# author-hidden-name/GAN-segmentation

Hardware: AMD Instinct MI355X
Metric: synthetic (image,mask) pairs/sec, FFHQ-1024 StyleGAN+decoder (higher is better)
Workload: dtype f32; 1 GPU; stylegan-ffhq 1024^2 synthesis + 2-class decoder, batch=8 per GPU, fp32 (BASELINE.json configs[1]); synthetic weights/latents/noise; (img u8, mask u8) resident on rank 0; global_batch=8, parallelism=dp1, gather=none, backend=none, graph=eager (GSA_GRAPH=0)

## Files before the change

### gan-segmentation_amd/csrc/gsa_api.cpp

```cpp
#include <hip/hip_runtime.h>

#include <cmath>
#include <cstdarg>
#include <cstdio>
#include <cstdlib>
#include <cstring>
#include <map>
#include <string>
#include <vector>

#include "../../include/gsa.h"
#include "gsa_kernels.h"
#include "gsa_pack.h"

using namespace gsa;

namespace {

constexpr int kMaxLevels = 12;
thread_local std::string g_create_error;

struct HostTensor {
    std::vector<float> data;
    std::vector<int64_t> dims;
// ... 64 lines not shown
    int d_n = 0, d_s0 = 0, d_bn = 1;
    int d_feat[kMaxLevels + 1] = {0}, d_inch[kMaxLevels] = {0};
    std::map<std::string, HostTensor> dparams;
    DecLevelDev dl[kMaxLevels];

    int max_batch = 0;
    float* lat[2] = {nullptr, nullptr};
    float* styles = nullptr;
    float *t_raw = nullptr, *x1 = nullptr;
    float* x2[kMaxLevels] = {nullptr};
    Aff* aff1 = nullptr;
    Aff* aff2[kMaxLevels] = {nullptr};
    StatPart* partials = nullptr;
    StatPart* stat_acc = nullptr;
    unsigned* stat_tickets = nullptr;
    unsigned* map_ctl = nullptr;
    unsigned long long* map_ll[2] = {nullptr, nullptr};
    float* zeros = nullptr;
    unsigned long long* stamps = nullptr;
    float* din[kMaxLevels] = {nullptr};
    float* cvt[kMaxLevels] = {nullptr};
    float *ya[kMaxLevels] = {nullptr}, *scb[kMaxLevels] = {nullptr}, *prev[kMaxLevels] = {nullptr};

    hipStream_t side = nullptr;
    hipEvent_t ev_level[kMaxLevels] = {nullptr};
    hipEvent_t ev_fork = nullptr, ev_join = nullptr;
    int bf16 = 0;
    int prio = 0;
    int dbg = 0;
    int side_levels = -1;
// ... 261 lines not shown
int gsa_create(int device, gsa_ctx** out) {
    if (!out) return fail(nullptr, GSA_ERR_INVALID, "gsa_create: out is null");
    int count = 0;
    hipError_t e = hipGetDeviceCount(&count);
    if (e != hipSuccess || count <= 0)
        return fail(nullptr, GSA_ERR_HIP, "no HIP device available (%s)", e == hipSuccess ? "device count is 0" : hipGetErrorString(e));
    if (device < 0 || device >= count) return fail(nullptr, GSA_ERR_INVALID, "device %d out of range (%d devices)", device, count);
    e = hipSetDevice(device);
    if (e != hipSuccess) return fail(nullptr, GSA_ERR_HIP, "hipSetDevice(%d): %s", device, hipGetErrorString(e));
    gsa_ctx* c = new gsa_ctx();
    c->device = device;
    e = hipStreamCreateWithFlags(&c->side, hipStreamNonBlocking);
    for (int i = 0; e == hipSuccess && i < kMaxLevels; ++i) e = hipEventCreateWithFlags(&c->ev_level[i], hipEventDisableTiming);
    if (e == hipSuccess) e = hipEventCreateWithFlags(&c->ev_fork, hipEventDisableTiming);
    if (e == hipSuccess) e = hipEventCreateWithFlags(&c->ev_join, hipEventDisableTiming);
    if (e != hipSuccess) {
        const int rc = fail(nullptr, GSA_ERR_HIP, "creating the side stream: %s", hipGetErrorString(e));
        delete c;
        return rc;
    }
    if (e == hipSuccess) e = hipMalloc((void**)&c->zeros, 256);
    if (e == hipSuccess) e = hipMemset(c->zeros, 0, 256);
    if (e != hipSuccess) {
        const int rc = fail(nullptr, GSA_ERR_HIP, "allocating the zero page: %s", hipGetErrorString(e));
        delete c;
        return rc;
    }
    c->side_levels = env_int("GSA_SIDE_LEVELS", c->side_levels);
    c->dbg = env_int("GSA_DBG", c->dbg);
    c->prio = env_int("GSA_PRIO", c->prio);
// ... 1 lines not shown
    return GSA_OK;
}

void gsa_destroy(gsa_ctx* c) {
    if (!c) return;
    (void)hipSetDevice(c->device);
    (void)hipDeviceSynchronize();
    free_all(c->g_allocs);
    free_all(c->d_allocs);
    free_all(c->ws_allocs);
    for (auto& ev : c->prof_events) { (void)hipEventDestroy(ev.a); (void)hipEventDestroy(ev.b); }
    for (auto e : c->event_pool) (void)hipEventDestroy(e);
    for (int i = 0; i < kMaxLevels; ++i) if (c->ev_level[i]) (void)hipEventDestroy(c->ev_level[i]);
    if (c->ev_fork) (void)hipEventDestroy(c->ev_fork);
    if (c->ev_join) (void)hipEventDestroy(c->ev_join);
    if (c->side) (void)hipStreamDestroy(c->side);
    if (c->zeros) (void)hipFree(c->zeros);
    delete c;
}

const char* gsa_last_error(const gsa_ctx* c) { return c ? c->err.c_str() : g_create_error.c_str(); }


int gsa_generator_init(gsa_ctx* c, const gsa_generator_config* g) {
    if (!c || !g) return GSA_ERR_INVALID;
    if (g->max_res_log2 < 2 || g->max_res_log2 > kMaxLevels) return fail(c, GSA_ERR_INVALID, "max_res_log2 %d out of range", g->max_res_log2);
    if (g->latent_size != 512) return fail(c, GSA_ERR_INVALID, "latent_size must be 512 (latent_avg is (512,) in the reference)");
    if (g->channels < 1 || g->channels > 4) return fail(c, GSA_ERR_INVALID, "channels must be 1..4");
    c->gc = *g;
    c->nlev = g->max_res_log2 - 1;
// ... 303 lines not shown
            for (int nb = 1; nb <= max_batch; ++nb)
                prow_elems = std::max(prow_elems, (size_t)conv_stat_rows((int)R, (int)R, (int)C, nb) * C);
            prow_elems = std::max(prow_elems, (size_t)post_prow((int)R, (int)R, (int)C) * C);
        }
        if (int rc = dev_alloc(c, N * maxact, &c->t_raw, T)) return rc;
        if (int rc = dev_alloc(c, N * maxact, &c->x1, T)) return rc;
        if (int rc = dev_alloc(c, N * maxC, &c->aff1, T)) return rc;
        prow_elems = std::max(prow_elems, (size_t)64 * maxC);
        if (int rc = dev_alloc_zeroed(c, N * prow_elems, &c->partials, T)) return rc;
        c->partials_bytes = N * prow_elems * sizeof(StatPart);
        c->stat_acc_bytes = N * maxC * sizeof(StatPart);
        c->ticket_bytes = N * ((maxC + 63) / 64) * sizeof(unsigned);
        c->stats_dirty = false;
        if (int rc = dev_alloc_zeroed(c, N * maxC, &c->stat_acc, T)) return rc;
        if (int rc = dev_alloc_zeroed(c, N * ((maxC + 63) / 64), &c->stat_tickets, T)) return rc;
    }
    if (int rc = dev_alloc_zeroed(c, 16, &c->stamps, T)) return rc;
    if (c->d_ready) {
        for (int i = c->d_s0; i < c->d_n; ++i) {
            const DecLevelDev& d = c->dl[i];
            const size_t R = (size_t)4 << i;
            if (int rc = dev_alloc(c, N * R * R * d.I, &c->din[i], T)) return rc;
            if (int rc = dev_alloc(c, N * R * R * d.F, &c->cvt[i], T)) return rc;
            if (!d.is_last) {
                if (int rc = dev_alloc(c, N * 4 * R * R * d.cs, &c->ya[i], T)) return rc;
                if (int rc = dev_alloc(c, N * 4 * R * R * d.cs, &c->prev[i], T)) return rc;
                if (d.has_sc)
                    if (int rc = dev_alloc(c, N * (2 * R >= 16 ? 1 : 4) * R * R * d.cs, &c->scb[i], T)) return rc;
            }
        }
// ... 35 lines not shown
        if (int rc = run_mapping(c, s, n, z, c->lat[0])) return rc;
        const float* w = c->lat[0];
        Launch lp(c, s, "g.styles", 2.0 * N * L * c->style_cols, 4.0 * ((double)L * c->style_cols + N * c->style_cols));
        HIP_TRY(launch_styles(w, c->latent_avg, c->psi, c->style_wt, c->style_b, c->style_col_layer, c->styles, n, L, c->style_cols, s));
    } else {
        Launch lp(c, s, "g.styles", 2.0 * N * L * c->style_cols, 4.0 * ((double)L * c->style_cols + N * 2 * nlev * L + N * c->style_cols));
        HIP_TRY(launch_styles_dlatents(dl, c->latent_avg, c->psi, c->style_wt, c->style_b, c->style_tiles, c->style_num_tiles, c->styles, n, L,
                                       c->style_cols, 2 * nlev, s));
    }

    char layer[64];
    for (int l = 0; l < nlev; ++l) {
        const GenBlockDev& B = c->blk[l];
        const int R = B.R, C = B.C, Cin = B.Cin;
        const double px = N * R * R;
        for (int k = 0; k < 2; ++k) {
            const float* nz = noise[2 * l + k];
            if (!nz) return fail(c, GSA_ERR_INVALID, "noise plane %d is null", 2 * l + k);
            int prow = 0;
            if (k == 0) {
                PostParams pp{};
                pp.noise = nz; pp.nscale = B.nscale[0]; pp.nbias = B.nbias[0];
                pp.out = c->x1; pp.partials = c->partials; pp.H = R; pp.W = R; pp.C = C; pp.bf16 = c->bf16;
                if (!B.has_conv1) {
                    pp.src = c->constant; pp.src_per_sample = 0; pp.blur = nullptr;
                } else {
                    ConvParams cp = conv_base(c);
                    cp.src0 = c->x2[l - 1]; cp.aff0 = c->aff2[l - 1]; cp.C0 = Cin;
                    cp.Hs = R / 2; cp.Ws = R / 2; cp.H = R; cp.W = R;
                    cp.wpk = B.w1; cp.Cout = C; cp.out = c->t_raw;
// ... 9 lines not shown
                    }
                    pp.src = c->t_raw; pp.src_per_sample = 1; pp.blur = B.blur;
                }
                snprintf(layer, sizeof layer, "g.%d.post_1", R);
                if (post_fuses_finalize(pp)) {
                    FinalizeParams fp{};
                    fp.partials = c->partials; fp.prow = 0; fp.HW = R * R; fp.C = C; fp.acc = c->stat_acc; fp.tickets = c->stat_tickets;
                    fp.style = c->styles + B.style_off[0]; fp.style_stride = c->style_cols;
                    fp.gamma = B.gamma[0]; fp.beta = B.beta[0];
                    fp.aff = c->aff1;
                    fp.flags = c->map_ctl;
                    Launch lp(c, s, layer, 0.0, 4.0 * (2 * px * C + px));
                    HIP_TRY(launch_post_fin(pp, fp, n, s));
                    continue;
                }
                Launch lp(c, s, layer, 0.0, 4.0 * (2 * px * C + px));
#ifdef GSA_DBG_HOOKS
                if (!((c->dbg & 8) && R >= 512))
#endif
                HIP_TRY(launch_post(pp, n, s));
                prow = post_rows_used(pp);
            } else {
                ConvParams cp = conv_base(c);
                cp.src0 = c->x1; cp.aff0 = c->aff1; cp.C0 = C;
                cp.Hs = R; cp.Ws = R; cp.H = R; cp.W = R;
                cp.wpk = B.w2; cp.wino = B.w2u; cp.Cout = C; cp.out = c->x2[l];
                cp.noise = nz; cp.nscale = B.nscale[1]; cp.nbias = B.nbias[1]; cp.partials = c->partials;
                snprintf(layer, sizeof layer, "g.%d.conv_2", R);
                int rows = conv_stat_rows(R, R, C, n);
                cp.stat_rows_host = &rows;
                const bool fused_fin = conv_fuses_finalize(cp, EPI_SYNTH, false);
                const double products = conv_form_products(conv3x3_form(cp, EPI_SYNTH, false));
                if (fused_fin) {
                    cp.fin_style = c->styles + B.style_off[1]; cp.fin_style_stride = c->style_cols;
                    cp.fin_gamma = B.gamma[1]; cp.fin_beta = B.beta[1]; cp.fin_aff = c->aff2[l]; cp.fin_flags = c->map_ctl;
                }
                Launch lp(c, s, layer, 2.0 * px * C * C * products, 4.0 * (2 * px * C + px), 2.0 * px * C * C * 9);
                HIP_TRY(launch_conv3x3(cp, EPI_SYNTH, false, n, s));
                prow = rows;
                if (fused_fin) continue;
            }
            if (c->fault == 2 && l == 3 && k == 1) {
// ... 214 lines not shown
    const float* fsrc[kMaxLevels];
    const Aff* faff[kMaxLevels];
    for (int l = 0; l < c->nlev; ++l) { fsrc[l] = c->x2[l]; faff[l] = c->aff2[l]; }
    const int want = c->side_levels < 0 ? c->d_n - 1 : c->side_levels;
    const int ns = want > c->d_n - 1 ? c->d_n - 1 : want;
    if (ns > 0) {
        HIP_TRY(hipEventRecord(c->ev_fork, s));
        HIP_TRY(hipStreamWaitEvent(c->side, c->ev_fork, 0));
    }
    bool fuse_rgb = false;
    if (img && ns <= c->d_n - 1 && factor == 1) {
        const int last = c->d_n - 1;
        ConvParams cp = cvt_params(c, last, fsrc[last], faff[last]);
        fuse_rgb = conv_fuses_torgb(cp, EPI_DEC, false, c->gc.channels);
    }
    if (int rc = run_generator(c, s, n, z, dl, noise, nullptr, fuse_rgb || factor > 1 ? nullptr : img, nullptr, ns > 0)) return rc;
    if (img && factor > 1) {
        const int l = c->nlev - 1, R = c->blk[l].R, C = c->blk[l].C, nc = c->gc.channels;
        const double px = (double)n * R * R;
        Launch lp(c, s, "g.torgb_down", 2.0 * px * C * nc, px * 4.0 * C + px / (factor * factor) * nc);
        HIP_TRY(launch_torgb_down(c->x2[l], c->aff2[l], c->rgb_w, c->rgb_b, img, n, R, R, C, nc, factor, c->bf16, s));
    }
    if (ns > 0) {
        if (int rc = run_decoder(c, c->side, n, fsrc, faff, nullptr, nullptr, 0, ns, true)) return rc;
        HIP_TRY(hipEventRecord(c->ev_join, c->side));
        HIP_TRY(hipStreamWaitEvent(s, c->ev_join, 0));
    }
    return run_decoder(c, s, n, fsrc, faff, nullptr, mask, ns, -1, false, fuse_rgb ? img : nullptr, factor);
}

int gsa_generate(gsa_ctx* c, void* stream, int32_t n, const float* z, const float* const* noise, int32_t num_noise, uint8_t* img,
// ... 135 lines not shown
```

### gan-segmentation_amd/csrc/gsa_dev.h

```cpp
#pragma once
#include "gsa_kernels.h"

#ifndef GSA_NO_XCD_REMAP
#define GSA_NO_XCD_REMAP 0
#endif

namespace gsa {

#ifdef GSA_STAMP
#define GSA_DBG_HOOKS 1
#endif
#ifdef GSA_STAMP
#define STAMP(i) do { __builtin_amdgcn_sched_barrier(0); asm volatile("s_memtime %0\n\ts_waitcnt lgkmcnt(0)" : "=s"(stamp_t[i]) :: "memory"); __builtin_amdgcn_sched_barrier(0); } while (0)
#define STAMP_DECL unsigned long long stamp_t[8] = {0, 0, 0, 0, 0, 0, 0, 0}
#define STAMP_FLUSH(nph) do { if (p.stamps && (threadIdx.x & 63) == 0) { for (int i_ = 0; i_ < (nph); ++i_) atomicAdd(&p.stamps[i_], stamp_t[i_ + 1] - stamp_t[i_]); atomicAdd(&p.stamps[15], 1ull); } } while (0)
#define TICK(var) do { __builtin_amdgcn_sched_barrier(0); asm volatile("s_memtime %0\n\ts_waitcnt lgkmcnt(0)" : "=s"(var) :: "memory"); __builtin_amdgcn_sched_barrier(0); } while (0)
#define TSUM(acc, a, b) acc += (b) - (a)
#define TFLUSH(idx, acc) do { if (p.stamps && (threadIdx.x & 63) == 0) atomicAdd(&p.stamps[idx], acc); } while (0)
#else
#define TICK(var) do {} while (0)
#define TSUM(acc, a, b) do {} while (0)
#define TFLUSH(idx, acc) do {} while (0)
#define STAMP(i) do {} while (0)
#define STAMP_DECL do {} while (0)
#define STAMP_FLUSH(nph) do {} while (0)
#endif


constexpr int kDirectRows = 64;

typedef float f32x4 __attribute__((ext_vector_type(4)));
typedef float f32x2 __attribute__((ext_vector_type(2)));
typedef __bf16 bf16x2 __attribute__((ext_vector_type(2)));
typedef unsigned u32x4 __attribute__((ext_vector_type(4)));
typedef short s16x4 __attribute__((ext_vector_type(4)));


__device__ __forceinline__ float max1(float a, float b) { float r; asm("v_max_f32 %0, %1, %2" : "=v"(r) : "v"(a), "v"(b)); return r; }
__device__ __forceinline__ float lrelu(float v) { return max1(v, 0.2f * v); }

__device__ __forceinline__ unsigned long long to_fixed(float v, double scale) {
    const double magic = 6755399441055744.0;
    double t = fma((double)v, scale, magic);
    return (unsigned long long)__double_as_longlong(t) - (unsigned long long)__double_as_longlong(magic);
}

__device__ __forceinline__ int stat_s2(int HW) {
    const int s2 = 40 - (HW > 1 ? 32 - __builtin_clz((unsigned)HW - 1u) : 0);
    return s2 < 20 ? 20 : (s2 > 26 ? 26 : s2);
}
__device__ __forceinline__ double stat_scale2(int HW) { return __hiloint2double((1023 + stat_s2(HW)) << 20, 0); }
__device__ __forceinline__ unsigned long long to_fixed_sq(float q, int s2) {
    const bool big = q >= __int_as_float((127 + 50 - s2) << 23);
    const float qs = big ? q * __int_as_float((127 + 20 - s2) << 23) : q;
    const unsigned long long k = to_fixed(qs, __hiloint2double((1023 + s2) << 20, 0));
    return k << (big ? s2 - 20 : 0);
}

template <int CTRL>
__device__ __forceinline__ float dpp_quad(float v) {
    return __int_as_float(__builtin_amdgcn_mov_dpp(__float_as_int(v), CTRL, 0xF, 0xF, true));
}

__device__ __forceinline__ f32x4 quad_transpose(float v0, float v1, float v2, float v3, int j) {
    const bool b0 = (j & 1) != 0, b1 = (j & 2) != 0;
    float pa = dpp_quad<0xB1>(v0), pb = dpp_quad<0xB1>(v1);
    const float a0 = b0 ? pb : v0, a1 = b0 ? v1 : pa;
    pa = dpp_quad<0xB1>(v2); pb = dpp_quad<0xB1>(v3);
    const float a2 = b0 ? pb : v2, a3 = b0 ? v3 : pa;
    pa = dpp_quad<0x4E>(a0); pb = dpp_quad<0x4E>(a2);
    const float c0 = b1 ? pb : a0, c2 = b1 ? a2 : pa;
// ... 113 lines not shown
```

### gan-segmentation_amd/csrc/gsa_kernels.h

```cpp
#pragma once
#include <hip/hip_runtime.h>
#include <stdint.h>
#include <stdlib.h>

#include <atomic>
#include <string>

namespace gsa {

struct Aff { float mean, A, B, pad; };

struct StatPart { unsigned long long s1, s2; };

constexpr double kStatScale1 = 268435456.0;

enum Epilogue { EPI_RAW = 0, EPI_SYNTH = 1, EPI_DEC = 2 };

struct ConvParams {
    int device;
    const float* src0; const Aff* aff0; int C0;
    const float* src1; int C1;
    int Hs, Ws;
    int up;
    int H, W;
    const float* wpk;
    const float* wino;
    int Cout;
// ... 4 lines not shown
    const float* resid; int resid_up;
    const float* resid1; int res_c0;
    const float* wsc; const float* sc_bias; float* out_sc;
    int tiles_x, tiles_y, groups, total_tiles;
    int stats_direct;
    int* stat_rows_host;
    int w_resident;
    int group_minor;
    unsigned long long* stamps;
    int dbg;
    int prio;
    int bf16;
    const float* fin_style; int fin_style_stride; const float* fin_gamma; const float* fin_beta; Aff* fin_aff; unsigned* fin_flags;
    const float* zeros;
    const float* rgb_w; const float* rgb_b; uint8_t* rgb_img;
};

struct PostParams {
    const float* src;
    int src_per_sample;
    const float* blur;
    const float* noise; const float* nscale; const float* nbias;
    float* out; StatPart* partials; int prow;
    int H, W, C;
    int bf16;
    int row_groups;
};

struct FinalizeParams {
    const StatPart* partials; int prow; int HW; int C;
// ... 12 lines not shown


enum class ConvForm { Wino43, WinoDma, WinoTwoTiles, WinoLean, Wino, KSplit, Bf16Lean, Direct };
ConvForm conv3x3_form(const ConvParams& p, int epi, bool shortcut);
hipError_t launch_conv3x3(const ConvParams& p, int epi, bool shortcut, int n, hipStream_t s);
inline bool conv_form_wino(ConvForm f) { return f <= ConvForm::Wino; }
inline double conv_form_products(ConvForm f) { return f == ConvForm::Wino43 ? 2.25 : conv_form_wino(f) ? 4 : 9; }
inline bool wino_shape(int H, int Cout, int bf16) { return !bf16 && (H >= 64 || (H >= 32 && Cout >= 64) || (H >= 16 && Cout >= 256)); }
inline bool wino43_shape(int H, int Cin) { return Cin >= 64 && H >= 32; }
bool wino43_enabled();
bool wino_lean_applies(const ConvParams& p, int epi);
bool wino_stream_paired(const ConvParams& p, int n);
hipError_t launch_wino_lean(const ConvParams& p, int epi, int n, hipStream_t s);
bool wino_lean_fuses_torgb(const ConvParams& p, int epi, int nc);
bool conv_fuses_torgb(const ConvParams& p, int epi, bool shortcut, int nc);
bool bf16_lean_applies(const ConvParams& p, int epi, bool shortcut);
hipError_t launch_bf16_lean(const ConvParams& p, int epi, int n, hipStream_t s);
bool subpixel_lean_applies(const ConvParams& p, int nt, int epi, bool sc, int kb, bool wst);
hipError_t launch_subpixel_lean(const ConvParams& q, int nt, int epi, bool sc, int kb, bool wst, dim3 grid, hipStream_t s);
enum class SubPath { Resident, Streamed, Plain };
struct SubpixelPlan {
    int ct;
    SubPath path;
    bool wino;
    int kb;
    size_t lds;
    int wgs_per_group;
};
SubpixelPlan subpixel_plan(const ConvParams& p, bool shortcut, int n);
hipError_t launch_subpixel(const ConvParams& p, int epi, bool shortcut, int n, hipStream_t s);
// ... 82 lines not shown
```

### gan-segmentation_amd/csrc/gsa_kernels.hip

```cpp
#include "gsa_kernels.h"
#include "gsa_dev.h"

#include <cxxabi.h>

#include <cstdio>
#include <cstdlib>
#include <cstring>
#include <mutex>
#include <vector>

#ifndef GSA_MFMA_PRIO
#define GSA_MFMA_PRIO 2
#endif
#ifndef GSA_OPERAND_PIPELINE
#define GSA_OPERAND_PIPELINE 1
#endif
#ifndef GSA_NO_XCD_REMAP
#define GSA_NO_XCD_REMAP 0
#endif
#ifndef GSA_POST_OCC
#define GSA_POST_OCC 2
#endif
#ifndef GSA_WINO_SOA
#define GSA_WINO_SOA 0
// ... 2648 lines not shown
    if ((int)gridDim.x > p.prow) {
        for (int i = threadIdx.x; i < p.C; i += 256) {
            StatPart* a = p.partials + ((size_t)n * p.prow + (blockIdx.x & (kDirectRows - 1))) * p.C + i;
            atomicAdd(&a->s1, sstat[i]);
            atomicAdd(&a->s2, sstat[p.C + i]);
        }
        return;
    }
    for (int i = threadIdx.x; i < p.C; i += 256) {
        StatPart sp; sp.s1 = sstat[i]; sp.s2 = sstat[p.C + i];
        p.partials[((size_t)n * p.prow + blockIdx.x) * p.C + i] = sp;
    }
}

__device__ __forceinline__ void finalize_one(const FinalizeParams& p, int n, int c, unsigned long long I1, unsigned long long I2) {
    const double inv_hw = 1.0 / (double)p.HW;
    const double m = (double)(long long)I1 * (1.0 / kStatScale1) * inv_hw;
    const double e2 = (double)(long long)I2 * (1.0 / stat_scale2(p.HW)) * inv_hw;
    double var = fma(-m, m, e2);
    {
        const long long s1 = (long long)I1;
        const bool near_wrap = (s1 < 0 ? -s1 : s1) >= (1ll << 61) || I2 >= (1ull << 61);
        if (p.flags && (near_wrap || var < -1e-6 * (e2 + m * m) - 1e-30)) atomicOr(p.flags, 1u);
    }
    if (!(var > 0.0)) var = 0.0;
    const float mean_f = (float)m, var_f = (float)var;
    const float inv = 1.0f / sqrtf(var_f + 1e-5f);
    const float gsc = p.gamma[c] * inv;
    const float* st = p.style + (size_t)n * p.style_stride;
    const float s1 = st[c] + 1.0f;
    Aff a;
    a.mean = mean_f;
    a.A = gsc * s1;
    a.B = fmaf(-mean_f, a.A, fmaf(p.beta[c], s1, st[p.C + c]));
    a.pad = 0.0f;
    p.aff[(size_t)n * p.C + c] = a;
}

__global__ __launch_bounds__(256) void finalize_kernel(FinalizeParams p, int rows_per_block) {
    __shared__ unsigned long long sh[2][256];
    __shared__ int is_last;
    const int n = blockIdx.y;
    const int cblk = p.C >= 64 ? 64 : p.C, nrg = 256 / cblk;
    const int cl = threadIdx.x % cblk, rg = threadIdx.x / cblk;
    const int c = blockIdx.x * 64 + cl;
    unsigned long long I1 = 0, I2 = 0;
    if (rg < nrg && c < p.C) {
        const int r0 = blockIdx.z * rows_per_block;
        const int r1 = min(p.prow, r0 + rows_per_block);
        const StatPart* base = p.partials + (size_t)n * p.prow * p.C + c;
#pragma unroll 16
// ... 928 lines not shown
}

ConvForm conv3x3_form(const ConvParams& p, int epi, bool sc) {
    if (wino_rule(p, epi, sc)) {
        if (wino43_enabled() && wino43_shape(p.H, p.C0) && p.resid == nullptr) return ConvForm::Wino43;
        if (wino_dma(p, epi) && wino_nt(p) == 1) return ConvForm::WinoDma;
        if (wino_tw(p) == 2) return ConvForm::WinoTwoTiles;
        return wino_lean_applies(p, epi) ? ConvForm::WinoLean : ConvForm::Wino;
    }
    if (ksplit_rule(p, sc)) return ConvForm::KSplit;
    return bf16_lean_applies(p, epi, sc) ? ConvForm::Bf16Lean : ConvForm::Direct;
}

hipError_t launch_conv3x3(const ConvParams& p, int epi, bool sc, int n, hipStream_t s) {
    if (p.H != p.W || (p.H & (p.H - 1)) || p.H < 4 || p.Cout % 16 || p.C0 % 16 || p.C1 % 16) return hipErrorInvalidValue;
    switch (conv3x3_form(p, epi, sc)) {
#if GSA_EXPERIMENTS
        case ConvForm::Wino43: return launch_wino43(p, epi, n, s);
        case ConvForm::WinoDma: return launch_wino_dma(p, epi, n, s);
        case ConvForm::WinoTwoTiles: return launch_wino_two_tiles(p, epi, n, s);
#endif
        case ConvForm::WinoLean: return launch_wino_lean(p, epi, n, s);
        case ConvForm::Wino: return launch_wino(p, epi, n, s);
        case ConvForm::KSplit: return launch_ksplit(p, epi, n, s);
        case ConvForm::Bf16Lean: return launch_bf16_lean(p, epi, n, s);
        case ConvForm::Direct: return launch_direct(p, epi, sc, n, s);
        default: return hipErrorInvalidValue;
    }
}

static bool fuse_finalize() {
    static const bool enabled = env_int("GSA_FUSEFIN", 1) != 0;
    return enabled;
}
bool conv_fuses_finalize(const ConvParams& p, int epi, bool sc) {
    return fuse_finalize() && epi == EPI_SYNTH && p.H <= 8 && conv3x3_form(p, epi, sc) == ConvForm::KSplit;
}

bool conv_fuses_torgb(const ConvParams& p, int epi, bool sc, int nc) {
    return conv3x3_form(p, epi, sc) == ConvForm::WinoLean && wino_lean_fuses_torgb(p, epi, nc);
}

bool subpixel_uses_wino(const ConvParams& p) {
    static const bool enabled = env_int("GSA_WINO22", 1) != 0;
    return enabled && !p.bf16;
}

SubpixelPlan subpixel_plan(const ConvParams& p, bool sc, int n) {
    static const bool res_enabled = env_int("GSA_SUBRES", 1) != 0;
    static const bool wst_enabled = env_int("GSA_SUBWST", 1) != 0;
    SubpixelPlan plan{};
    plan.wino = subpixel_uses_wino(p);
    const long tiles = (long)(p.H / 16) * (p.W / 16) * n;
    plan.ct = 16;
    for (int ct = plan.wino ? 32 : 64; ct > 16; ct /= 2)
// ... 270 lines not shown
```

### gan-segmentation_amd/csrc/gsa_wino_lean.hip

```cpp
#include "gsa_kernels.h"
#include "gsa_dev.h"

#include <cstdio>
#include <cstdlib>
#include <type_traits>

namespace gsa {
namespace lean {

constexpr int LH = 18, LW = 18, RS = LW * 16 + 4;
constexpr int IMG = LH * RS;
constexpr int SEG = 16 * 256;
constexpr int NPIX = LH * LW;

struct Tile { int n, y0, x0; };

template <int EPI, bool AFF, bool RES, int NB, int GW, bool DB = true, int PF = 1, bool RGB = false>
__global__ __launch_bounds__(256 * GW, GW == 1 ? (DB ? 2 : 3) : 1) void conv3x3_wino_lean(ConvParams p) {
    static_assert(!RGB || (NB == 1 && GW == 1 && DB && AFF && EPI == EPI_DEC), "fused toRGB: the 16 -> 16 decoder kernel with an AdaIN source");
    static_assert(DB || (NB == 1 && GW == 1), "single-buffered form: one block, one group");
    static_assert(PF == 1 || (PF == 2 && DB), "two prefetch sets: the double-buffered form");
    constexpr int NTHR = 256 * GW, CIN = 16 * NB, COUT = 16 * GW;
    constexpr int NCH = (NPIX * 4 + NTHR - 1) / NTHR;
    constexpr bool kLastPartial = (NPIX * 4) % NTHR != 0;
    extern __shared__ __attribute__((aligned(16))) float smem[];
    float* const sA = smem;
    float* const sB = smem + (DB ? 2 : 1) * IMG;
    const int tid = threadIdx.x, lane = tid & 63;
    const int wave8 = __builtin_amdgcn_readfirstlane(tid >> 6);
    const int wave = wave8 & 3, gsel = wave8 >> 2;
    const int i16 = lane & 15, kq = lane >> 4, part = tid & 3;
    const int H = p.H, W = p.W;
    const int per = (p.total_tiles + (int)gridDim.x - 1) / (int)gridDim.x;
    const int w_begin = xcd_block(blockIdx.x, gridDim.x) * per;
    const int w_end = min(p.total_tiles, w_begin + per);
    if (w_begin >= w_end) return;
// ... 37 lines not shown
        if (e) {
#pragma unroll
            for (int k = 0; k < NCH; ++k) {
                const unsigned bad = (eflags >> (4 * k)) & (unsigned)e;
                const unsigned off = s_off[k] + (bad ? safe_off - s_off[k] : 0u);
                ra[S][k] = *reinterpret_cast<const f32x4*>(hb + off);
            }
        } else {
#pragma unroll
            for (int k = 0; k < NCH; ++k) ra[S][k] = *reinterpret_cast<const f32x4*>(hb + s_off[k]);
        }
    };
    auto write_item = [&](auto set_tag, const Tile& t, int e, int cb, int buf) {
        constexpr int S = decltype(set_tag)::value;
        float* img = sA + buf * IMG;
        if (AFF && t.n != n_coef) {
#pragma unroll
            for (int h = 0; h < NB; ++h) {
                const f32x4* a = reinterpret_cast<const f32x4*>(p.aff0 + (size_t)t.n * CIN + h * 16 + part * 4);
                const f32x4 a0 = a[0], a1 = a[1], a2 = a[2], a3 = a[3];
                cA[h] = f32x4{a0[1], a1[1], a2[1], a3[1]};
                cB[h] = f32x4{a0[2], a1[2], a2[2], a3[2]};
            }
            n_coef = t.n;
        }
        const f32x4 kA = NB == 1 || cb == 0 ? cA[0] : cA[NB - 1], kB = NB == 1 || cb == 0 ? cB[0] : cB[NB - 1];
        const f32x4 z = {0.f, 0.f, 0.f, 0.f};
        if (e) {
#pragma unroll
            for (int k = 0; k < NCH; ++k) {
                const f32x4 v = AFF ? fma4(ra[S][k], kA, kB) : ra[S][k];
// ... 268 lines not shown
            __syncthreads();
            if (has_next) write_item(S0{}, tr, er, 0, 0);
            epilogue_loads(tc);
            Tile t2 = tr; int e2c = er, cb2 = 0;
            if (it + 2 < items) { next_item(t2, e2c, cb2); load_item(S0{}, t2, e2c, cb2); }
            mfmas(std::true_type{}, 0);
            loads_landed(ra[0], acc[15]);
            epilogue(tc);
            if (EPI == EPI_SYNTH && (!has_next || tr.n != tc.n)) flush_stats(tc.n);
            __syncthreads();
            tc = tr; ec = er; tr = t2; er = e2c;
        }
    }
}

__device__ unsigned g_cu_tickets[4096];
__device__ __forceinline__ void antiphase_start(int cycles64, float* lds_word) {
    if (cycles64 <= 0) return;
    if (threadIdx.x == 0) {
        unsigned hw, xcc;
        asm volatile("s_getreg_b32 %0, hwreg(HW_REG_HW_ID)" : "=s"(hw));
        asm volatile("s_getreg_b32 %0, hwreg(HW_REG_XCC_ID)" : "=s"(xcc));
        const unsigned cu = ((xcc & 15u) << 8) | (((hw >> 13) & 7u) << 5) | (((hw >> 12) & 1u) << 4) | ((hw >> 8) & 15u);
        *reinterpret_cast<unsigned*>(lds_word) = atomicAdd(&g_cu_tickets[cu & 4095u], 1u);
    }
    __syncthreads();
    const unsigned ticket = *reinterpret_cast<volatile unsigned*>(lds_word);
    __syncthreads();
    if (ticket & 1u)
        for (int i = 0; i < cycles64; i += 16) __builtin_amdgcn_s_sleep(16);
}

template <int EPI, bool AFF, int NT, int IL, bool PAIR>
__device__ __forceinline__ void wino_stream_body(const ConvParams& p) {
    static_assert(!PAIR || (NT == 1 && IL == 0), "paired form: one group per wave quad, phased memory instructions");
    constexpr int NTHR = PAIR ? 512 : 256;
    constexpr int NCH = (NPIX * 4 + NTHR - 1) / NTHR;
    constexpr int NP = PAIR ? 2 : NT;
    extern __shared__ __attribute__((aligned(16))) float smem[];
    float* const sA = smem;
    float* const sB = smem + 2 * IMG;
    float* const sE = sB + 2 * NP * SEG;
    float* const sC = sE + 64 * NP;
    const int tid = threadIdx.x, lane = tid & 63;
    const int wave8 = __builtin_amdgcn_readfirstlane(tid >> 6);
    const int wave = PAIR ? wave8 & 3 : wave8;
    const int quad = PAIR ? wave8 >> 2 : 0;
    const int i16 = lane & 15, kq = lane >> 4, part = tid & 3;
    const int H = p.H, W = p.W, CIN = p.C0, COUT = p.Cout, nblk = p.C0 >> 4;
    const int g = PAIR ? 2 * (int)blockIdx.y + quad : (int)blockIdx.y;
// ... 47 lines not shown
        if ((p.dbg & 512) && dbg_items > 2) return;
#endif
        if (e) {
#pragma unroll
            for (int k = 0; k < NCH; ++k) {
                const unsigned bad = (eflags >> (4 * k)) & (unsigned)e;
                const unsigned off = s_off[k] + (bad ? safe_off - s_off[k] : 0u);
                ra[k] = *reinterpret_cast<const f32x4*>(hb + off);
            }
        } else {
#pragma unroll
            for (int k = 0; k < NCH; ++k) ra[k] = *reinterpret_cast<const f32x4*>(hb + s_off[k]);
        }
    };
    int n_coef = -1;
    auto coefficients = [&](int n) {
        __syncthreads();
        for (int e = tid; e < CIN; e += NTHR) {
            const f32x4 a = *reinterpret_cast<const f32x4*>(p.aff0 + (size_t)n * CIN + e);
            sC[(e >> 4) * 32 + (e & 15)] = a[1];
            sC[(e >> 4) * 32 + 16 + (e & 15)] = a[2];
        }
        __syncthreads();
    };
    auto write_item = [&](const Tile& t, int e, int cb, int buf) {
        float* img = sA + buf * IMG;
        if (AFF && t.n != n_coef) { coefficients(t.n); n_coef = t.n; }
#ifdef GSA_DBG_HOOKS
        if (++dbg_items > 2 && (p.dbg & 128)) return;
#endif
        f32x4 kA = {0.f, 0.f, 0.f, 0.f}, kB = kA;
        if (AFF) {
            kA = *reinterpret_cast<const f32x4*>(sC + cb * 32 + part * 4);
            kB = *reinterpret_cast<const f32x4*>(sC + cb * 32 + 16 + part * 4);
        }
        const f32x4 z = {0.f, 0.f, 0.f, 0.f};
        if (e) {
#pragma unroll
            for (int k = 0; k < NCH; ++k) {
                const f32x4 v = AFF ? fma4(ra[k], kA, kB) : ra[k];
                const bool bad = ((eflags >> (4 * k)) & (unsigned)e) != 0;
                if (k < NCH - 1 || l_off[NCH - 1] >= 0) *reinterpret_cast<f32x4*>(img + l_off[k]) = bad ? z : v;
// ... 243 lines not shown
    }
    TFLUSH(6, sw); TFLUSH(7, sl); TFLUSH(8, sm); TFLUSH(9, se); TFLUSH(10, sb);
    TFLUSH(12, (unsigned long long)items); TFLUSH(15, 1ull);
}

template <int EPI, bool AFF, int NT = 1, int IL = 0>
__global__ __launch_bounds__(256, NT == 1 ? 2 : 1) void conv3x3_wino_stream(ConvParams p) {
    wino_stream_body<EPI, AFF, NT, IL, false>(p);
}

template <int EPI, bool AFF>
__global__ __launch_bounds__(512, 1) void conv3x3_wino_stream_pair(ConvParams p) {
    wino_stream_body<EPI, AFF, 1, 0, true>(p);
}

template <int EPI, bool AFF, bool RES, int NB, int GW, bool DB = true, int PF = 1, bool RGB = false>
hipError_t launch_t(const ConvParams& p, int n, hipStream_t s) {
    const size_t lds = sizeof(float) * ((DB ? 2 : 1) * IMG + GW * NB * SEG);
    const int cus = device_cus(p.device);
    ConvParams q = p;
    q.wpk = p.wino;
    q.tiles_x = p.W / 16;
    q.tiles_y = p.H / 16;
    q.groups = 1;
    q.total_tiles = q.tiles_x * q.tiles_y * n;
    if (EPI == EPI_SYNTH) {
        q.stats_direct = 1;
        q.prow = kDirectRows;
        if (p.stat_rows_host) *p.stat_rows_host = q.prow;
    }
    const int gx = std::min(q.total_tiles, cus * (GW == 1 ? (DB ? 2 : 3) : 1));
    return launch<conv3x3_wino_lean<EPI, AFF, RES, NB, GW, DB, PF, RGB>>(p.device, dim3(gx), dim3(256 * GW), lds, s, q);
}

bool single_buffered() {
    static const bool on = env_int("GSA_WINO_LEAN_SB", 0) != 0;
    return on;
}

int prefetch_sets() {
    static const int pf = env_int("GSA_WINO_LEAN_PF", 1);
    return pf == 2 ? 2 : 1;
}

template <int NB, int GW>
hipError_t launch_shape(const ConvParams& p, int epi, int n, hipStream_t s) {
// ... 37 lines not shown
    q.groups = p.Cout / (16 * NP);
#if GSA_EXPERIMENTS
    static const int stagger = env_int("GSA_STAGGER", 0);
    q.group_minor = PAIR ? 0 : stagger;
#else
    q.group_minor = 0;
#endif
    q.total_tiles = q.tiles_x * q.tiles_y * n;
    if (EPI == EPI_SYNTH) {
        q.stats_direct = 1;
        q.prow = kDirectRows;
        if (p.stat_rows_host) *p.stat_rows_host = q.prow;
    }
    const int slots = std::max(1, cus * (NP == 1 ? 2 : 1) / q.groups);
    const int gx = std::min(q.total_tiles, slots);
    if constexpr (PAIR) return launch<conv3x3_wino_stream_pair<EPI, AFF>>(p.device, dim3(gx, q.groups), dim3(512), lds, s, q);
    else return launch<conv3x3_wino_stream<EPI, AFF, NT, IL>>(p.device, dim3(gx, q.groups), dim3(256), lds, s, q);
}

}
using namespace lean;

bool wino_lean_applies(const ConvParams& p, int epi) {
    static const int enabled = env_int("GSA_WINO_LEAN", 7);
    if (p.H != p.W || p.H % 16) return false;
    if ((enabled & 4) && p.C0 >= 64 && p.C0 <= 512 && p.resid == nullptr && p.H >= 16)
        return epi == EPI_SYNTH ? (p.partials != nullptr && p.noise != nullptr && p.fin_aff == nullptr) : epi == EPI_DEC;
    const bool shape = (p.C0 == 16 && p.Cout == 16 && (enabled & 1)) || (p.C0 == 32 && p.Cout == 32 && (enabled & 2));
    if (!shape || p.H < 32) return false;
    if (epi == EPI_SYNTH) return p.partials != nullptr && p.noise != nullptr && p.fin_aff == nullptr && p.resid == nullptr;
// ... 24 lines not shown
#else
    (void)p; (void)n;
    return false;
#endif
}

int stream_interleaved() {
#if GSA_EXPERIMENTS
    static const int il = env_int("GSA_WINO_IL", 0);
    return il == 1 ? 1 : 0;
#else
    return 0;
#endif
}

hipError_t launch_wino_lean(const ConvParams& p, int epi, int n, hipStream_t s) {
    if (p.C0 >= 64) {
#if GSA_EXPERIMENTS
        if (stream_pairs(p, n)) {
            const int il = stream_interleaved();
#define GSA_STREAM2(IL_) \
            if (il == IL_) { \
                if (epi == EPI_SYNTH) return p.aff0 ? launch_stream_t<EPI_SYNTH, true, 2, IL_>(p, n, s) : launch_stream_t<EPI_SYNTH, false, 2, IL_>(p, n, s); \
                if (epi == EPI_DEC) return p.aff0 ? launch_stream_t<EPI_DEC, true, 2, IL_>(p, n, s) : launch_stream_t<EPI_DEC, false, 2, IL_>(p, n, s); \
                return hipErrorInvalidValue; \
            }
            GSA_STREAM2(0) GSA_STREAM2(1)
#undef GSA_STREAM2
            return hipErrorInvalidValue;
        }
#endif
// ... 16 lines not shown
```

Measured before the change: 1424 pairs/s.

## Fuse AdaIN stat finalization into the following Winograd conv for synth conv_2

For generator levels of 64 and up, the post kernel after conv_1 now writes per-sample statistic rows to a dedicated zeroed buffer. The next Winograd conv reduces those rows in LDS and computes the AdaIN affine coefficients itself, so the separate finalize step between the two convolutions is skipped. The buffer is zeroed on a side stream at call start and the main stream waits on an event before first use. The cost is redundant reduction work in every workgroup whenever the tile's sample changes, plus extra LDS atomics and kernel variants.

```diff
diff --git a/gan-segmentation_amd/csrc/gsa_api.cpp b/gan-segmentation_amd/csrc/gsa_api.cpp
--- a/gan-segmentation_amd/csrc/gsa_api.cpp
+++ b/gan-segmentation_amd/csrc/gsa_api.cpp
@@ -102,6 +102,12 @@
     StatPart* partials = nullptr;
     StatPart* stat_acc = nullptr;
     unsigned* stat_tickets = nullptr;
+    StatPart* rows1[kMaxLevels] = {nullptr};
+    StatPart* sum_rows = nullptr;
+    size_t sum_rows_bytes = 0;
+    hipEvent_t ev_rows = nullptr;
+    bool sums_call = false;
+    bool sums_wait = false;
     unsigned* map_ctl = nullptr;
     unsigned long long* map_ll[2] = {nullptr, nullptr};
     float* zeros = nullptr;
@@ -393,6 +399,7 @@
     for (int i = 0; e == hipSuccess && i < kMaxLevels; ++i) e = hipEventCreateWithFlags(&c->ev_level[i], hipEventDisableTiming);
     if (e == hipSuccess) e = hipEventCreateWithFlags(&c->ev_fork, hipEventDisableTiming);
     if (e == hipSuccess) e = hipEventCreateWithFlags(&c->ev_join, hipEventDisableTiming);
+    if (e == hipSuccess) e = hipEventCreateWithFlags(&c->ev_rows, hipEventDisableTiming);
     if (e != hipSuccess) {
         const int rc = fail(nullptr, GSA_ERR_HIP, "creating the side stream: %s", hipGetErrorString(e));
         delete c;
@@ -424,6 +431,7 @@
     for (int i = 0; i < kMaxLevels; ++i) if (c->ev_level[i]) (void)hipEventDestroy(c->ev_level[i]);
     if (c->ev_fork) (void)hipEventDestroy(c->ev_fork);
     if (c->ev_join) (void)hipEventDestroy(c->ev_join);
+    if (c->ev_rows) (void)hipEventDestroy(c->ev_rows);
     if (c->side) (void)hipStreamDestroy(c->side);
     if (c->zeros) (void)hipFree(c->zeros);
     delete c;
@@ -757,6 +765,16 @@
         c->stats_dirty = false;
         if (int rc = dev_alloc_zeroed(c, N * maxC, &c->stat_acc, T)) return rc;
         if (int rc = dev_alloc_zeroed(c, N * ((maxC + 63) / 64), &c->stat_tickets, T)) return rc;
+        size_t own_elems = 0;
+        for (int l = 0; l < c->nlev; ++l) { c->rows1[l] = nullptr; if (!c->bf16 && (4 << l) >= 64) own_elems += N * kDirectRows * (size_t)c->ch[l]; }
+        c->sum_rows = nullptr;
+        c->sum_rows_bytes = own_elems * sizeof(StatPart);
+        if (own_elems) {
+            if (int rc = dev_alloc_zeroed(c, own_elems, &c->sum_rows, T)) return rc;
+            size_t at = 0;
+            for (int l = 0; l < c->nlev; ++l)
+                if ((4 << l) >= 64) { c->rows1[l] = c->sum_rows + at; at += N * kDirectRows * (size_t)c->ch[l]; }
+        }
     }
     if (int rc = dev_alloc_zeroed(c, 16, &c->stamps, T)) return rc;
     if (c->d_ready) {
@@ -822,6 +840,13 @@
         const GenBlockDev& B = c->blk[l];
         const int R = B.R, C = B.C, Cin = B.Cin;
         const double px = N * R * R;
+        ConvParams cp2 = conv_base(c);
+        cp2.src0 = c->x1; cp2.aff0 = c->aff1; cp2.C0 = C;
+        cp2.Hs = R; cp2.Ws = R; cp2.H = R; cp2.W = R;
+        cp2.wpk = B.w2; cp2.wino = B.w2u; cp2.Cout = C; cp2.out = c->x2[l];
+        cp2.noise = noise[2 * l + 1]; cp2.nscale = B.nscale[1]; cp2.nbias = B.nbias[1]; cp2.partials = c->partials;
+        bool own1 = false;
+        int own1_rows = 0;
         for (int k = 0; k < 2; ++k) {
             const float* nz = noise[2 * l + k];
             if (!nz) return fail(c, GSA_ERR_INVALID, "noise plane %d is null", 2 * l + k);
@@ -861,18 +886,28 @@
                     HIP_TRY(launch_post_fin(pp, fp, n, s));
                     continue;
                 }
+                own1 = c->sums_call && c->rows1[l] != nullptr && post_rows_used(pp) <= kDirectRows && conv_reads_sums(cp2, EPI_SYNTH, false, n);
+                if (own1) {
+                    pp.partials = c->rows1[l];
+                    if (c->sums_wait) {
+                        HIP_TRY(hipStreamWaitEvent(s, c->ev_rows, 0));
+                        c->sums_wait = false;
+                    }
+                }
                 Launch lp(c, s, layer, 0.0, 4.0 * (2 * px * C + px));
 #ifdef GSA_DBG_HOOKS
                 if (!((c->dbg & 8) && R >= 512))
 #endif
                 HIP_TRY(launch_post(pp, n, s));
                 prow = post_rows_used(pp);
+                if (own1) { own1_rows = prow; continue; }
             } else {
-                ConvParams cp = conv_base(c);
-                cp.src0 = c->x1; cp.aff0 = c->aff1; cp.C0 = C;
-                cp.Hs = R; cp.Ws = R; cp.H = R; cp.W = R;
-                cp.wpk = B.w2; cp.wino = B.w2u; cp.Cout = C; cp.out = c->x2[l];
-                cp.noise = nz; cp.nscale = B.nscale[1]; cp.nbias = B.nbias[1]; cp.partials = c->partials;
+                ConvParams cp = cp2;
+                if (own1) {
+                    cp.in_rows = c->rows1[l]; cp.in_nrows = own1_rows; cp.in_HW = R * R;
+                    cp.in_style = c->styles + B.style_off[0]; cp.in_style_stride = c->style_cols;
+                    cp.in_gamma = B.gamma[0]; cp.in_beta = B.beta[0]; cp.in_flags = c->map_ctl;
+                }
                 snprintf(layer, sizeof layer, "g.%d.conv_2", R);
                 int rows = conv_stat_rows(R, R, C, n);
                 cp.stat_rows_host = &rows;
@@ -1117,7 +1152,20 @@
         ConvParams cp = cvt_params(c, last, fsrc[last], faff[last]);
         fuse_rgb = conv_fuses_torgb(cp, EPI_DEC, false, c->gc.channels);
     }
-    if (int rc = run_generator(c, s, n, z, dl, noise, nullptr, fuse_rgb || factor > 1 ? nullptr : img, nullptr, ns > 0)) return rc;
+    c->sums_call = fin_read_enabled() && c->sum_rows != nullptr && !c->bf16;
+    c->sums_wait = false;
+    if (c->sums_call) {
+        if (ns > 0) {
+            HIP_TRY(hipMemsetAsync(c->sum_rows, 0, c->sum_rows_bytes, c->side));
+            HIP_TRY(hipEventRecord(c->ev_rows, c->side));
+            c->sums_wait = true;
+        } else {
+            HIP_TRY(hipMemsetAsync(c->sum_rows, 0, c->sum_rows_bytes, s));
+        }
+    }
+    const int grc = run_generator(c, s, n, z, dl, noise, nullptr, fuse_rgb || factor > 1 ? nullptr : img, nullptr, ns > 0);
+    c->sums_call = c->sums_wait = false;
+    if (grc) return grc;
     if (img && factor > 1) {
         const int l = c->nlev - 1, R = c->blk[l].R, C = c->blk[l].C, nc = c->gc.channels;
         const double px = (double)n * R * R;
diff --git a/gan-segmentation_amd/csrc/gsa_dev.h b/gan-segmentation_amd/csrc/gsa_dev.h
--- a/gan-segmentation_amd/csrc/gsa_dev.h
+++ b/gan-segmentation_amd/csrc/gsa_dev.h
@@ -27,8 +27,6 @@
 #endif
 
 
-constexpr int kDirectRows = 64;
-
 typedef float f32x4 __attribute__((ext_vector_type(4)));
 typedef float f32x2 __attribute__((ext_vector_type(2)));
 typedef __bf16 bf16x2 __attribute__((ext_vector_type(2)));
@@ -55,6 +53,30 @@
     const float qs = big ? q * __int_as_float((127 + 20 - s2) << 23) : q;
     const unsigned long long k = to_fixed(qs, __hiloint2double((1023 + s2) << 20, 0));
     return k << (big ? s2 - 20 : 0);
+}
+
+__device__ __forceinline__ Aff finalize_coeffs(unsigned long long I1, unsigned long long I2, int HW, const float* gamma, const float* beta,
+                                               const float* st, int C, int c, unsigned* flags) {
+    const double inv_hw = 1.0 / (double)HW;
+    const double m = (double)(long long)I1 * (1.0 / kStatScale1) * inv_hw;
+    const double e2 = (double)(long long)I2 * (1.0 / stat_scale2(HW)) * inv_hw;
+    double var = fma(-m, m, e2);
+    {
+        const long long s1 = (long long)I1;
+        const bool near_wrap = (s1 < 0 ? -s1 : s1) >= (1ll << 61) || I2 >= (1ull << 61);
+        if (flags && (near_wrap || var < -1e-6 * (e2 + m * m) - 1e-30)) atomicOr(flags, 1u);
+    }
+    if (!(var > 0.0)) var = 0.0;
+    const float mean_f = (float)m, var_f = (float)var;
+    const float inv = 1.0f / sqrtf(var_f + 1e-5f);
+    const float gsc = gamma[c] * inv;
+    const float s1 = st[c] + 1.0f;
+    Aff a;
+    a.mean = mean_f;
+    a.A = gsc * s1;
+    a.B = fmaf(-mean_f, a.A, fmaf(beta[c], s1, st[C + c]));
+    a.pad = 0.0f;
+    return a;
 }
 
 template <int CTRL>
diff --git a/gan-segmentation_amd/csrc/gsa_kernels.h b/gan-segmentation_amd/csrc/gsa_kernels.h
--- a/gan-segmentation_amd/csrc/gsa_kernels.h
+++ b/gan-segmentation_amd/csrc/gsa_kernels.h
@@ -11,6 +11,7 @@
 struct Aff { float mean, A, B, pad; };
 
 struct StatPart { unsigned long long s1, s2; };
+constexpr int kDirectRows = 64;
 
 constexpr double kStatScale1 = 268435456.0;
 
@@ -45,6 +46,8 @@
     const float* fin_style; int fin_style_stride; const float* fin_gamma; const float* fin_beta; Aff* fin_aff; unsigned* fin_flags;
     const float* zeros;
     const float* rgb_w; const float* rgb_b; uint8_t* rgb_img;
+    const StatPart* in_rows; int in_nrows; int in_HW;
+    const float* in_style; int in_style_stride; const float* in_gamma; const float* in_beta; unsigned* in_flags;
 };
 
 struct PostParams {
@@ -87,6 +90,9 @@
 hipError_t launch_wino_lean(const ConvParams& p, int epi, int n, hipStream_t s);
 bool wino_lean_fuses_torgb(const ConvParams& p, int epi, int nc);
 bool conv_fuses_torgb(const ConvParams& p, int epi, bool shortcut, int nc);
+bool fin_read_enabled();
+bool wino_lean_reads_sums(const ConvParams& p, int epi, int n);
+bool conv_reads_sums(const ConvParams& p, int epi, bool shortcut, int n);
 bool bf16_lean_applies(const ConvParams& p, int epi, bool shortcut);
 hipError_t launch_bf16_lean(const ConvParams& p, int epi, int n, hipStream_t s);
 bool subpixel_lean_applies(const ConvParams& p, int nt, int epi, bool sc, int kb, bool wst);
diff --git a/gan-segmentation_amd/csrc/gsa_kernels.hip b/gan-segmentation_amd/csrc/gsa_kernels.hip
--- a/gan-segmentation_amd/csrc/gsa_kernels.hip
+++ b/gan-segmentation_amd/csrc/gsa_kernels.hip
@@ -2686,27 +2686,7 @@
 }
 
 __device__ __forceinline__ void finalize_one(const FinalizeParams& p, int n, int c, unsigned long long I1, unsigned long long I2) {
-    const double inv_hw = 1.0 / (double)p.HW;
-    const double m = (double)(long long)I1 * (1.0 / kStatScale1) * inv_hw;
-    const double e2 = (double)(long long)I2 * (1.0 / stat_scale2(p.HW)) * inv_hw;
-    double var = fma(-m, m, e2);
-    {
-        const long long s1 = (long long)I1;
-        const bool near_wrap = (s1 < 0 ? -s1 : s1) >= (1ll << 61) || I2 >= (1ull << 61);
-        if (p.flags && (near_wrap || var < -1e-6 * (e2 + m * m) - 1e-30)) atomicOr(p.flags, 1u);
-    }
-    if (!(var > 0.0)) var = 0.0;
-    const float mean_f = (float)m, var_f = (float)var;
-    const float inv = 1.0f / sqrtf(var_f + 1e-5f);
-    const float gsc = p.gamma[c] * inv;
-    const float* st = p.style + (size_t)n * p.style_stride;
-    const float s1 = st[c] + 1.0f;
-    Aff a;
-    a.mean = mean_f;
-    a.A = gsc * s1;
-    a.B = fmaf(-mean_f, a.A, fmaf(p.beta[c], s1, st[p.C + c]));
-    a.pad = 0.0f;
-    p.aff[(size_t)n * p.C + c] = a;
+    p.aff[(size_t)n * p.C + c] = finalize_coeffs(I1, I2, p.HW, p.gamma, p.beta, p.style + (size_t)n * p.style_stride, p.C, c, p.flags);
 }
 
 __global__ __launch_bounds__(256) void finalize_kernel(FinalizeParams p, int rows_per_block) {
@@ -3665,6 +3645,7 @@
 
 hipError_t launch_conv3x3(const ConvParams& p, int epi, bool sc, int n, hipStream_t s) {
     if (p.H != p.W || (p.H & (p.H - 1)) || p.H < 4 || p.Cout % 16 || p.C0 % 16 || p.C1 % 16) return hipErrorInvalidValue;
+    if (p.in_rows != nullptr && !conv_reads_sums(p, epi, sc, n)) return hipErrorInvalidValue;
     switch (conv3x3_form(p, epi, sc)) {
 #if GSA_EXPERIMENTS
         case ConvForm::Wino43: return launch_wino43(p, epi, n, s);
@@ -3690,6 +3671,10 @@
 
 bool conv_fuses_torgb(const ConvParams& p, int epi, bool sc, int nc) {
     return conv3x3_form(p, epi, sc) == ConvForm::WinoLean && wino_lean_fuses_torgb(p, epi, nc);
+}
+
+bool conv_reads_sums(const ConvParams& p, int epi, bool sc, int n) {
+    return conv3x3_form(p, epi, sc) == ConvForm::WinoLean && wino_lean_reads_sums(p, epi, n);
 }
 
 bool subpixel_uses_wino(const ConvParams& p) {
diff --git a/gan-segmentation_amd/csrc/gsa_wino_lean.hip b/gan-segmentation_amd/csrc/gsa_wino_lean.hip
--- a/gan-segmentation_amd/csrc/gsa_wino_lean.hip
+++ b/gan-segmentation_amd/csrc/gsa_wino_lean.hip
@@ -15,11 +15,46 @@
 
 struct Tile { int n, y0, x0; };
 
-template <int EPI, bool AFF, bool RES, int NB, int GW, bool DB = true, int PF = 1, bool RGB = false>
-__global__ __launch_bounds__(256 * GW, GW == 1 ? (DB ? 2 : 3) : 1) void conv3x3_wino_lean(ConvParams p) {
+
+template <int NTHR>
+__device__ __forceinline__ void coefficients_from_sums(const ConvParams& p, int n, int CIN, float* scratch, float* table, int tid) {
+    asm volatile("" : "+v"(tid));
+    unsigned long long* const acc = reinterpret_cast<unsigned long long*>(scratch);
+    __syncthreads();
+    for (int e = tid; e < 2 * CIN; e += NTHR) acc[e] = 0ull;
+    __syncthreads();
+    const u32x4* const rows = reinterpret_cast<const u32x4*>(p.in_rows + (size_t)n * p.in_nrows * CIN);
+    const int total = p.in_nrows * CIN;
+    for (int e0 = tid; e0 < total; e0 += 4 * NTHR) {
+        u32x4 r[4];
+#pragma unroll
+        for (int j = 0; j < 4; ++j) r[j] = e0 + j * NTHR < total ? rows[e0 + j * NTHR] : u32x4{0u, 0u, 0u, 0u};
+#pragma unroll
+        for (int j = 0; j < 4; ++j) {
+            const int e = e0 + j * NTHR;
+            if (e < total) {
+                const int ch = e % CIN;
+                atomicAdd(&acc[2 * ch], ((unsigned long long)r[j][1] << 32) | r[j][0]);
+                atomicAdd(&acc[2 * ch + 1], ((unsigned long long)r[j][3] << 32) | r[j][2]);
+            }
+        }
+    }
+    __syncthreads();
+    for (int e = tid; e < CIN; e += NTHR) {
+        const Aff a = finalize_coeffs(acc[2 * e], acc[2 * e + 1], p.in_HW, p.in_gamma, p.in_beta, p.in_style + (size_t)n * p.in_style_stride,
+                                      CIN, e, p.in_flags);
+        table[(e >> 4) * 32 + (e & 15)] = a.A;
+        table[(e >> 4) * 32 + 16 + (e & 15)] = a.B;
+    }
+    __syncthreads();
+}
+
+template <int EPI, bool AFF, bool RES, int NB, int GW, bool DB, int PF, bool RGB, bool SUMS>
+__device__ __forceinline__ void wino_lean_body(const ConvParams& p) {
     static_assert(!RGB || (NB == 1 && GW == 1 && DB && AFF && EPI == EPI_DEC), "fused toRGB: the 16 -> 16 decoder kernel with an AdaIN source");
     static_assert(DB || (NB == 1 && GW == 1), "single-buffered form: one block, one group");
     static_assert(PF == 1 || (PF == 2 && DB), "two prefetch sets: the double-buffered form");
+    static_assert(!SUMS || (AFF && DB), "sums-taking form: an AdaIN source; the image buffer being staged is the scratch");
     constexpr int NTHR = 256 * GW, CIN = 16 * NB, COUT = 16 * GW;
     constexpr int NCH = (NPIX * 4 + NTHR - 1) / NTHR;
     constexpr bool kLastPartial = (NPIX * 4) % NTHR != 0;
@@ -87,7 +122,19 @@
     auto write_item = [&](auto set_tag, const Tile& t, int e, int cb, int buf) {
         constexpr int S = decltype(set_tag)::value;
         float* img = sA + buf * IMG;
-        if (AFF && t.n != n_coef) {
+        if constexpr (SUMS) {
+            if (t.n != n_coef) {
+                float* const tab = img + 4 * CIN;
+                coefficients_from_sums<NTHR>(p, t.n, CIN, img, tab, tid);
+#pragma unroll
+                for (int h = 0; h < NB; ++h) {
+                    cA[h] = *reinterpret_cast<const f32x4*>(tab + h * 32 + part * 4);
+                    cB[h] = *reinterpret_cast<const f32x4*>(tab + h * 32 + 16 + part * 4);
+                }
+                __syncthreads();
+                n_coef = t.n;
+            }
+        } else if (AFF && t.n != n_coef) {
 #pragma unroll
             for (int h = 0; h < NB; ++h) {
                 const f32x4* a = reinterpret_cast<const f32x4*>(p.aff0 + (size_t)t.n * CIN + h * 16 + part * 4);
@@ -386,6 +433,23 @@
     }
 }
 
+template <int EPI, bool AFF, bool RES, int NB, int GW, bool DB = true, int PF = 1, bool RGB = false>
+__global__ __launch_bounds__(256 * GW, GW == 1 ? (DB ? 2 : 3) : 1) void conv3x3_wino_lean(ConvParams p) {
+    wino_lean_body<EPI, AFF, RES, NB, GW, DB, PF, RGB, false>(p);
+}
+
+}
+namespace sums {
+namespace lean {
+template <int EPI, bool AFF, bool RES, int NB, int GW, bool DB = true, int PF = 1, bool RGB = false>
+__global__ __launch_bounds__(256 * GW, GW == 1 ? 2 : 1) void conv3x3_wino_lean(ConvParams p) {
+    static_assert(AFF && !RES && DB && PF == 1 && !RGB, "the forms that have a sums-taking twin");
+    gsa::lean::wino_lean_body<EPI, AFF, RES, NB, GW, DB, PF, RGB, true>(p);
+}
+}
+}
+namespace lean {
+
 __device__ unsigned g_cu_tickets[4096];
 __device__ __forceinline__ void antiphase_start(int cycles64, float* lds_word) {
     if (cycles64 <= 0) return;
@@ -403,9 +467,10 @@
         for (int i = 0; i < cycles64; i += 16) __builtin_amdgcn_s_sleep(16);
 }
 
-template <int EPI, bool AFF, int NT, int IL, bool PAIR>
+template <int EPI, bool AFF, int NT, int IL, bool PAIR, bool SUMS = false>
 __device__ __forceinline__ void wino_stream_body(const ConvParams& p) {
     static_assert(!PAIR || (NT == 1 && IL == 0), "paired form: one group per wave quad, phased memory instructions");
+    static_assert(!SUMS || AFF, "sums-taking form: an AdaIN source");
     constexpr int NTHR = PAIR ? 512 : 256;
     constexpr int NCH = (NPIX * 4 + NTHR - 1) / NTHR;
     constexpr int NP = PAIR ? 2 : NT;
@@ -483,7 +548,11 @@
         }
     };
     int n_coef = -1;
-    auto coefficients = [&](int n) {
+    auto coefficients = [&](int n, float* img) {
+        if constexpr (SUMS) {
+            coefficients_from_sums<NTHR>(p, n, CIN, img, sC, tid);
+            return;
+        }
         __syncthreads();
         for (int e = tid; e < CIN; e += NTHR) {
             const f32x4 a = *reinterpret_cast<const f32x4*>(p.aff0 + (size_t)n * CIN + e);
@@ -494,7 +563,7 @@
     };
     auto write_item = [&](const Tile& t, int e, int cb, int buf) {
         float* img = sA + buf * IMG;
-        if (AFF && t.n != n_coef) { coefficients(t.n); n_coef = t.n; }
+        if (AFF && t.n != n_coef) { coefficients(t.n, img); n_coef = t.n; }
 #ifdef GSA_DBG_HOOKS
         if (++dbg_items > 2 && (p.dbg & 128)) return;
 #endif
@@ -768,6 +837,23 @@
     wino_stream_body<EPI, AFF, 1, 0, true>(p);
 }
 
+}
+namespace sums {
+namespace lean {
+template <int EPI, bool AFF, int NT = 1, int IL = 0>
+__global__ __launch_bounds__(256, 2) void conv3x3_wino_stream(ConvParams p) {
+    static_assert(AFF && NT == 1 && IL == 0, "the forms that have a sums-taking twin");
+    gsa::lean::wino_stream_body<EPI, AFF, NT, IL, false, true>(p);
+}
+template <int EPI, bool AFF>
+__global__ __launch_bounds__(512, 1) void conv3x3_wino_stream_pair(ConvParams p) {
+    static_assert(AFF, "the forms that have a sums-taking twin");
+    gsa::lean::wino_stream_body<EPI, AFF, 1, 0, true, true>(p);
+}
+}
+}
+namespace lean {
+
 template <int EPI, bool AFF, bool RES, int NB, int GW, bool DB = true, int PF = 1, bool RGB = false>
 hipError_t launch_t(const ConvParams& p, int n, hipStream_t s) {
     const size_t lds = sizeof(float) * ((DB ? 2 : 1) * IMG + GW * NB * SEG);
@@ -784,6 +870,11 @@
         if (p.stat_rows_host) *p.stat_rows_host = q.prow;
     }
     const int gx = std::min(q.total_tiles, cus * (GW == 1 ? (DB ? 2 : 3) : 1));
+    if (p.in_rows != nullptr) {
+        if constexpr (EPI == EPI_SYNTH && AFF && !RES && DB && PF == 1 && !RGB)
+            return launch<sums::lean::conv3x3_wino_lean<EPI, AFF, RES, NB, GW, DB, PF, RGB>>(p.device, dim3(gx), dim3(256 * GW), lds, s, q);
+        return hipErrorInvalidValue;
+    }
     return launch<conv3x3_wino_lean<EPI, AFF, RES, NB, GW, DB, PF, RGB>>(p.device, dim3(gx), dim3(256 * GW), lds, s, q);
 }
 
@@ -851,6 +942,13 @@
     }
     const int slots = std::max(1, cus * (NP == 1 ? 2 : 1) / q.groups);
     const int gx = std::min(q.total_tiles, slots);
+    if (p.in_rows != nullptr) {
+        if constexpr (EPI == EPI_SYNTH && AFF && NT == 1 && IL == 0) {
+            if constexpr (PAIR) return launch<sums::lean::conv3x3_wino_stream_pair<EPI, AFF>>(p.device, dim3(gx, q.groups), dim3(512), lds, s, q);
+            else return launch<sums::lean::conv3x3_wino_stream<EPI, AFF, NT, IL>>(p.device, dim3(gx, q.groups), dim3(256), lds, s, q);
+        }
+        return hipErrorInvalidValue;
+    }
     if constexpr (PAIR) return launch<conv3x3_wino_stream_pair<EPI, AFF>>(p.device, dim3(gx, q.groups), dim3(512), lds, s, q);
     else return launch<conv3x3_wino_stream<EPI, AFF, NT, IL>>(p.device, dim3(gx, q.groups), dim3(256), lds, s, q);
 }
@@ -905,7 +1003,18 @@
 #endif
 }
 
+bool fin_read_enabled() {
+    static const bool enabled = env_int("GSA_FIN_READ", 1) != 0;
+    return enabled;
+}
+bool wino_lean_reads_sums(const ConvParams& p, int epi, int n) {
+    if (!fin_read_enabled() || epi != EPI_SYNTH || p.aff0 == nullptr || p.bf16 || !wino_lean_applies(p, epi)) return false;
+    if (p.C0 >= 64) return p.C0 <= 512 && !stream_pairs(p, n);
+    return prefetch_sets() == 1;
+}
+
 hipError_t launch_wino_lean(const ConvParams& p, int epi, int n, hipStream_t s) {
+    if (p.in_rows != nullptr && (!wino_lean_reads_sums(p, epi, n) || p.in_nrows < 1 || p.in_nrows > kDirectRows)) return hipErrorInvalidValue;
     if (p.C0 >= 64) {
 #if GSA_EXPERIMENTS
         if (stream_pairs(p, n)) {
```

Result: no change. 1433 pairs/s (median of 6 runs) (+0.6%).
